# NVlabs/few-shot-vid2vid

Hardware: AMD Instinct MI355X
Metric: frames/sec G+D fwd+bwd step, 512x512 fewshot_pose (higher is better)
Workload: dtype f32; 1 GPU; fewshot_pose 512x512, per-GPU batch 2, adaptive_spade+warp_ref+spade_combine, D step + G step (train.py:58-62), Adam included, no VGG / no FlowNet2 / face-D; global_batch=2, parallelism=dp1, launch=hipgraph

## Files before the change

few-shot-vid2vid_amd/csrc/conv_igemm.hip:

```cpp
#include <stdlib.h>
#include "conv_igemm.h"


__device__ __forceinline__ void fsv_xcd_tile(int nx, int ny, int& bx, int& by) {
  const int b = blockIdx.x + blockIdx.y * nx;
  if ((nx & 7) != 0 || ny == 1) { bx = blockIdx.x; by = blockIdx.y; return; }
  const int xcd = b & 7, j = b >> 3;
  by = j % ny;
  bx = xcd + 8 * (j / ny);
}

template <int BM, int BN, int WM, int WN, int PF, bool AF, int DBG = 0, int MODE = 0, bool UP = false>
__device__ __forceinline__ void fsv_conv_igemm_body(const ConvP& p, const int bx, const int by, const int bz) {
  constexpr bool LD = MODE == 2, WT = MODE >= 1;
  constexpr int BK = FSV_BK;
  constexpr int NT = 64 * WM * WN;
  constexpr int RPA = NT / 8;
  constexpr int TM = BM / (WM * 32), TN = BN / (WN * 32);
  constexpr int NPA = BM / RPA;
  constexpr int QB = BN / 4;
  constexpr int RPB = NT / QB;
  constexpr int NPB = BK / RPB;
  constexpr int A_ST = BM * BK, B_ST = BK * BN;
  static_assert(TM >= 1 && TN >= 1 && NPA >= 1 && NPA * RPA == BM && NPB >= 1 && NPB * RPB == BK, "tile / thread-count mismatch");
// ... 974 lines not shown
      areg[i][0] = fsv_buf_load1(abuf, ok ? (unsigned)(((((long long)n * p.H + iy) * p.W + ix) * p.Cin + ci) * 4) : FSV_BUF_OOB);
    }
#pragma unroll
    for (int i = 0; i < NPB; ++i) {
      int m = pc * BK + bpr0 + i * RPB;
      bool rok = m < p.Mz;
      if (cout4) {
        breg[i] = fsv_buf_load4(bbuf, (rok && bcol < p.Cout) ? (unsigned)((m * p.Cout + bcol) * 4) : FSV_BUF_OOB);
      } else {
        const unsigned e = (unsigned)((m * p.Cout + bcol) * 4);
        breg[i] = make_float4(fsv_buf_load1(bbuf, (rok && bcol + 0 < p.Cout) ? e : FSV_BUF_OOB),
                              fsv_buf_load1(bbuf, (rok && bcol + 1 < p.Cout) ? e + 4 : FSV_BUF_OOB),
                              fsv_buf_load1(bbuf, (rok && bcol + 2 < p.Cout) ? e + 8 : FSV_BUF_OOB),
                              fsv_buf_load1(bbuf, (rok && bcol + 3 < p.Cout) ? e + 12 : FSV_BUF_OOB));
      }
    }
  };
  auto store_chunk = [&]() {
#pragma unroll
    for (int i = 0; i < NPA; ++i) {
      int pr = apr0 + i * RPA;
#pragma unroll
      for (int j = 0; j < V; ++j) As[pr * BMK + aq * V + j] = areg[i][j];
    }
#pragma unroll
    for (int i = 0; i < NPB; ++i) {
      int pr = bpr0 + i * RPB;
      *reinterpret_cast<float4*>(&Bs[pr * BN + bq * 4]) = breg[i];
    }
  };

  f32x16 acc[TM][TN];
#pragma unroll
  for (int i = 0; i < TM; ++i)
#pragma unroll
    for (int j = 0; j < TN; ++j)
#pragma unroll
      for (int r = 0; r < 16; ++r) acc[i][j][r] = 0.f;

  const int lrow = lane & 31, lk = lane >> 5;
  const float* a_frag = &As[lk * BMK + wm * (TM * 32) + lrow];
  const float* b_frag = &Bs[lk * BN + wn * (TN * 32) + lrow];
  if (c_begin < c_end) {
    load_chunk(c_begin);
    store_chunk();
    __syncthreads();
#pragma unroll 1
    for (int pc = c_begin; pc < c_end; ++pc) {
      const int pnext = (pc + 1 < c_end) ? pc + 1 : pc;
      load_chunk(pnext);
      float a[2][TM], b[2][TN];
#pragma unroll
      for (int i = 0; i < TM; ++i) a[0][i] = a_frag[i * 32];
#pragma unroll
      for (int j = 0; j < TN; ++j) b[0][j] = b_frag[j * 32];
#pragma unroll
      for (int kk = 0; kk < BK / 2; ++kk) {
        const int cur = kk & 1, nxt = cur ^ 1;
        if (kk + 1 < BK / 2) {
#pragma unroll
          for (int i = 0; i < TM; ++i) a[nxt][i] = a_frag[(kk + 1) * 2 * BMK + i * 32];
#pragma unroll
          for (int j = 0; j < TN; ++j) b[nxt][j] = b_frag[(kk + 1) * 2 * BN + j * 32];
        }
#pragma unroll
        for (int i = 0; i < TM; ++i)
#pragma unroll
          for (int j = 0; j < TN; ++j)
            acc[i][j] = __builtin_amdgcn_mfma_f32_32x32x2f32(a[cur][i], b[cur][j], acc[i][j], 0, 0, 0);
      }
      __syncthreads();
      store_chunk();
      __syncthreads();
    }
  }
#pragma unroll
  for (int j = 0; j < TN; ++j) {
    const int co = bn0 + wn * (TN * 32) + j * 32 + lrow;
    if (co >= p.Cout) continue;
#pragma unroll
    for (int i = 0; i < TM; ++i)
#pragma unroll
      for (int r = 0; r < 16; ++r) {
        const int row = (r & 3) + 8 * (r >> 2) + 4 * lk;
        const int k = bi0 + wm * (TM * 32) + i * 32 + row;
        if (k >= p.K) continue;
        float* dst = dwt + (long long)k * p.ldw + co;
        if (p.nsplit > 1) atomicAdd(dst, acc[i][j][r]); else *dst = acc[i][j][r];
      }
  }
}

#define FSV_THIN_MAXK 1152
template <int CO>
__global__ __launch_bounds__(256) void fsv_conv_thin_fwd_kernel(ConvP p, int iters) {
  __shared__ float wl[FSV_THIN_MAXK * CO];
  const int tid = threadIdx.x, lane = tid & 63, wave = tid >> 6;
  for (int i = tid; i < p.K * CO; i += 256) {
    const int k = i / CO, c = i - k * CO;
    wl[i] = (c < p.Cout) ? p.wt[(long long)k * p.ldw + c] : 0.f;
  }
  __syncthreads();
  const int QC = p.Cin >> 2;
  const int PPW = 64 / QC;
  const int cq = lane % QC, pl = lane / QC;
  const int ohw = p.OH * p.OW;
  const fsv_buf abuf = fsv_make_buf(p.in, (long long)p.N * p.H * p.W * p.Cin * 4);
  const float ws = p.wscale ? p.wscale[0] : 1.f;
  const int m_base = blockIdx.x * (4 * PPW * iters);
#pragma unroll 1
  for (int it = 0; it < iters; ++it) {
    const int m = m_base + (it * 4 + wave) * PPW + pl;
    const bool live = m < p.Mz;
    const int mm = live ? m : 0;
    const int n = mm / ohw, rem = mm - n * ohw;
    const int oy = rem / p.OW, ox = rem - oy * p.OW;
    float acc[CO];
#pragma unroll
    for (int c = 0; c < CO; ++c) acc[c] = 0.f;
#pragma unroll 3
    for (int t = 0; t < p.ntaps; ++t) {
      int ty, tx;
      fsv_tap(p, t, ty, tx);
      const int iy = oy * p.sy + ty, ix = ox * p.sx + tx;
      const bool ok = live & ((unsigned)iy < (unsigned)p.H) & ((unsigned)ix < (unsigned)p.W);
      const float4 v = fsv_buf_load4(abuf, ok ? (unsigned)((((n * p.H + iy) * p.W + ix) * p.Cin + cq * 4) * 4) : FSV_BUF_OOB);
      const float* w0 = wl + (t * p.Cin + cq * 4) * CO;
#pragma unroll
      for (int c = 0; c < CO; ++c) {
        acc[c] = fmaf(v.x, w0[c], acc[c]);
        acc[c] = fmaf(v.y, w0[CO + c], acc[c]);
        acc[c] = fmaf(v.z, w0[2 * CO + c], acc[c]);
        acc[c] = fmaf(v.w, w0[3 * CO + c], acc[c]);
      }
    }
    for (int o = 1; o < QC; o <<= 1) {
#pragma unroll
      for (int c = 0; c < CO; ++c) acc[c] += __shfl_xor(acc[c], o);
    }
    if (live && cq == 0) {
#pragma unroll
      for (int c = 0; c < CO; ++c) {
        if (c >= p.Cout) break;
        float v = acc[c] * ws;
        v = (v + (p.bias ? p.bias[c] : 0.f)) * p.scale;
        v = fsv_act(v, p.act);
        if (p.res) v += p.res[(long long)m * p.Cout + c];
        p.out[(long long)m * p.Cout + c] = v;
      }
    }
  }
}

template <int CO>
__global__ __launch_bounds__(256) void fsv_conv_thin_wgrad_kernel(WgradP p, int chunk) {
  __shared__ float red[256 * 4 * CO];
  const int QK = p.ntaps * (p.Cin >> 2);
  const int NG = 256 / QK;
  const int tid = threadIdx.x;
  const int q = tid % QK, g = tid / QK;
  const bool lane_on = g < NG;
  const int t = q / (p.Cin >> 2), ci = (q - t * (p.Cin >> 2)) * 4;
  int ty, tx;
  {
    unsigned long long code = (t < 8) ? p.taps_lo : p.taps_hi;
    int sh = (t & 7) * 8;
    ty = (int)((code >> sh) & 15ull) - 8;
    tx = (int)((code >> (sh + 4)) & 15ull) - 8;
  }
  const fsv_buf abuf = fsv_make_buf(p.in, (long long)p.N * p.H * p.W * p.Cin * 4);
  const fsv_buf dbuf = fsv_make_buf(p.dout, (long long)p.Mz * p.Cout * 4);
  const int ohw = p.OH * p.OW;
  const int m0 = blockIdx.x * chunk;
  const int m1 = (m0 + chunk < p.Mz) ? m0 + chunk : p.Mz;
  float acc[4][CO];
#pragma unroll
  for (int e = 0; e < 4; ++e)
#pragma unroll
    for (int c = 0; c < CO; ++c) acc[e][c] = 0.f;
  if (lane_on) {
#pragma unroll 4
    for (int m = m0 + g; m < m1; m += NG) {
      const int n = m / ohw, rem = m - n * ohw;
      const int oy = rem / p.OW, ox = rem - oy * p.OW;
      const int iy = oy * p.sy + ty, ix = ox * p.sx + tx;
      const bool ok = ((unsigned)iy < (unsigned)p.H) & ((unsigned)ix < (unsigned)p.W);
      const float4 v = fsv_buf_load4(abuf, ok ? (unsigned)((((n * p.H + iy) * p.W + ix) * p.Cin + ci) * 4) : FSV_BUF_OOB);
      float d[CO];
#pragma unroll
      for (int c = 0; c < CO; ++c) d[c] = fsv_buf_load1(dbuf, (c < p.Cout) ? (unsigned)((m * p.Cout + c) * 4) : FSV_BUF_OOB);
#pragma unroll
      for (int c = 0; c < CO; ++c) {
        acc[0][c] = fmaf(v.x, d[c], acc[0][c]);
        acc[1][c] = fmaf(v.y, d[c], acc[1][c]);
        acc[2][c] = fmaf(v.z, d[c], acc[2][c]);
        acc[3][c] = fmaf(v.w, d[c], acc[3][c]);
      }
    }
  }
#pragma unroll
  for (int e = 0; e < 4; ++e)
#pragma unroll
    for (int c = 0; c < CO; ++c) red[(e * CO + c) * 256 + tid] = acc[e][c];
  __syncthreads();
  if (g == 0) {
#pragma unroll
    for (int e = 0; e < 4; ++e)
#pragma unroll
      for (int c = 0; c < CO; ++c) {
        float s = 0.f;
        for (int gg = 0; gg < NG; ++gg) s += red[(e * CO + c) * 256 + gg * QK + q];
        if (c < p.Cout) atomicAdd(p.dwt + (long long)(t * p.Cin + ci + e) * p.ldw + c, s);
      }
  }
}

static inline bool fsv_conv_thin(int Mz, int K) {
  const int sw = (int)fsv_env("FSV_CONV_THIN", 1);
  if (sw == 0) return false;
  if (sw == 2) return true;
  return K <= 1152 && (long long)Mz >= 64ll * K;
}

__global__ __launch_bounds__(256) void fsv_prep_weight_kernel(const float* w, float* wt, const float* scale_ptr,
                                                              const float* col_scale,
                                                              int mode_in, int Cout, int Cin, int KH, int KW,
                                                              int ntaps, unsigned long long taps_lo,
                                                              unsigned long long taps_hi, int Kpad, int ldw,
                                                              long long w_bstride, long long wt_bstride) {
  const int z = blockIdx.z;
  const float s = scale_ptr ? *scale_ptr : 1.f;
  const long long total = (long long)Kpad * ldw;
  const bool accum = mode_in == 3;
  const int mode = accum ? 2 : mode_in;
  const int rowlen = (mode == 1) ? Cout : Cin;
  const int ncols = (mode == 1) ? Cin : Cout;
  const int K = ntaps * rowlen;
  long long i = (long long)blockIdx.x * 256 + threadIdx.x;
  const long long stride = (long long)gridDim.x * 256;
  for (; i < total; i += stride) {
    int r = (int)(i / ldw), c = (int)(i - (long long)r * ldw);
    bool ok = r < K && c < ncols;
    int j = ok ? r / rowlen : 0;
    int a = r - j * rowlen;
    unsigned long long code = (j < 8) ? taps_lo : taps_hi;
    int sh = (j & 7) * 8;
    int kh = (int)((code >> sh) & 15ull), kw = (int)((code >> (sh + 4)) & 15ull);
    int co = (mode == 1) ? a : c, ci = (mode == 1) ? c : a;
    long long widx = (((long long)co * Cin + ci) * KH + kh) * KW + kw + (long long)z * w_bstride;
    if (mode == 2) {
      if (ok) {
        float g = s * wt[(long long)z * wt_bstride + i];
        ((float*)w)[widx] = accum ? ((float*)w)[widx] + g : g;
      }
    } else {
      float v = 0.f;
      if (ok) v = col_scale ? w[widx] * col_scale[co] : s * w[widx];
      wt[(long long)z * wt_bstride + i] = v;
    }
  }
}

struct PrepGroup {
  const long long* src; const long long* dst; const int* dims; const unsigned long long* taps;
};
template <int KKT>
__device__ __forceinline__ void fsv_prep_stage(const PrepGroup& g, const int layer, const int cot, const int cit, float* t) {
  const int* d = g.dims + layer * 9;
  const int Cout = d[0], CinR = d[2], KW = d[4];
  const int KK = KKT ? KKT : d[3] * KW;
  const int CI_T = KK <= 8 ? 32 : 16;
  const int run = CI_T * KK, lds = run + 1;
  const float* w = reinterpret_cast<const float*>(g.src[layer]);
  const int co0 = cot * 32, ci0 = cit * CI_T;
  const int tid = threadIdx.x;
  const int total = 32 * run;
  constexpr int U = 8;
  for (int e0 = tid; e0 < total; e0 += 256 * U) {
    float val[U];
    int dst[U];
#pragma unroll
    for (int u = 0; u < U; ++u) {
      const int e = e0 + 256 * u;
      const int col = e / run, idx = e - col * run;
      const int co = co0 + col, ci = ci0 + idx / KK;
      const bool ok = (e < total) & (co < Cout) & (ci < CinR);
      val[u] = ok ? w[((long long)co * CinR + ci0) * KK + idx] : 0.f;
      dst[u] = (e < total) ? col * lds + idx : -1;
    }
#pragma unroll
    for (int u = 0; u < U; ++u)
      if (dst[u] >= 0) t[dst[u]] = val[u];
  }
}

__device__ __forceinline__ float fsv_prep_pick(const float* src, const int code, const int KW, const bool masked) {
  if (!masked) return src[(code & 15) * KW + (code >> 4)];
  const int mh = code & 15, mw = code >> 4;
  float s = 0.f;
  bool first = true;
  for (int kh = 0; kh < 4; ++kh) {
    if (!((mh >> kh) & 1)) continue;
    for (int kw = 0; kw < 4; ++kw) {
      if (!((mw >> kw) & 1)) continue;
      const float v = src[kh * KW + kw];
      s = first ? v : s + v;
      first = false;
    }
  }
  return s;
}

template <int KKT>
__device__ __forceinline__ void fsv_prep_emit(const PrepGroup& g, const int layer, const int cot, const int cit, const float* t) {
  const int* d = g.dims + layer * 9;
  const int Cout = d[0], CinP = d[1], KW = d[4], ntaps = d[5], ldw = d[7];
  const int mode = d[8] & 1;
  const bool masked = (d[8] & 4) != 0;
  const int KK = KKT ? KKT : d[3] * KW;
  const int CI_T = KK <= 8 ? 32 : 16;
  const int run = CI_T * KK, lds = run + 1;
  float* wt = reinterpret_cast<float*>(g.dst[layer]);
  const unsigned long long lo = g.taps[layer * 2], hi = g.taps[layer * 2 + 1];
  const int co0 = cot * 32, ci0 = cit * CI_T;
  const int tid = threadIdx.x;
  if (mode == 0) {
    const int q = tid & 7, r0 = tid >> 3;
    const int nrows = ntaps * CI_T;
    for (int r = r0; r < nrows; r += 32) {
      const int j = r / CI_T, cil = r - j * CI_T;
      const int ci = ci0 + cil;
      if (ci >= CinP) continue;
      const unsigned long long code8 = (j < 8) ? lo : hi;
      const int code = (int)((code8 >> ((j & 7) * 8)) & 255ull);
      const float* src = t + (4 * q) * lds + cil * KK;
      *reinterpret_cast<float4*>(&wt[((long long)j * CinP + ci) * ldw + co0 + 4 * q]) =
          make_float4(fsv_prep_pick(src, code, KW, masked), fsv_prep_pick(src + lds, code, KW, masked),
                      fsv_prep_pick(src + 2 * lds, code, KW, masked), fsv_prep_pick(src + 3 * lds, code, KW, masked));
    }
  } else {
    const int QN = CI_T / 4;
    const int q = tid % QN, r0 = tid / QN, rstep = 256 / QN;
    const int nrows = ntaps * 32;
    for (int r = r0; r < nrows; r += rstep) {
      const int j = r >> 5, col = r & 31;
      const int co = co0 + col, ci = ci0 + 4 * q;
      if (co >= Cout || ci >= CinP) continue;
      const unsigned long long code8 = (j < 8) ? lo : hi;
      const int code = (int)((code8 >> ((j & 7) * 8)) & 255ull);
      const float* src = t + col * lds + (4 * q) * KK;
      float* dstp = &wt[((long long)j * Cout + co) * ldw + ci];
      if (ci + 3 < CinP) {
        *reinterpret_cast<float4*>(dstp) =
            make_float4(fsv_prep_pick(src, code, KW, masked), fsv_prep_pick(src + KK, code, KW, masked),
                        fsv_prep_pick(src + 2 * KK, code, KW, masked), fsv_prep_pick(src + 3 * KK, code, KW, masked));
      } else {
        for (int k = 0; ci + k < CinP; ++k) dstp[k] = fsv_prep_pick(src + k * KK, code, KW, masked);
      }
    }
  }
}

template <int KKT>
__device__ __forceinline__ void fsv_prep_layer(const PrepGroup& g, const int first, const int njobs, const int cot, const int cit,
                                               float* t) {
  fsv_prep_stage<KKT>(g, first, cot, cit, t);
  __syncthreads();
  for (int j = 0; j < njobs; ++j) fsv_prep_emit<KKT>(g, first + j, cot, cit, t);
}

__global__ __launch_bounds__(256) void fsv_prep_group_kernel(PrepGroup g, const int* tmap) {
  __shared__ float t[32 * 257];
  const int first = tmap[blockIdx.x * 4], njobs = tmap[blockIdx.x * 4 + 1];
  const int cot = tmap[blockIdx.x * 4 + 2], cit = tmap[blockIdx.x * 4 + 3];
// ... 112 lines not shown
      FSV_CONV_TILES(FSV_V4_CASE)
      FSV_CONV_TILES_DIAG(FSV_V4_CASE)
#undef FSV_V4_CASE
      default: return FSV_ERR_BAD_ARG;
    }
  } else {
    switch (t->shape) {
#define FSV_V1_CASE(SHAPE, BM, BN, WM, WN) \
  case SHAPE: FSV_LAUNCH((fsv_conv_igemm_v1_kernel<BM, BN, WM, WN>), g, dim3(64 * WM * WN), stream, p); break;
      FSV_CONV_V1_SHAPES(FSV_V1_CASE)
#undef FSV_V1_CASE
      default: return FSV_ERR_BAD_ARG;
    }
  }
  return fsv_check_launch();
}

#include <stdlib.h>
#include <string.h>
static inline long long fsv_tune(int which) {
  static long long vals[4] = {-1, -1, -1, -1};
  if (vals[0] < 0) {
    vals[1] = (long long)fsv_env("FSV_SPLIT_TARGET", 512);
    vals[2] = (long long)fsv_env("FSV_WG_TARGET", 1024);
    vals[3] = (long long)fsv_env("FSV_WG_MINCH", 8);
    vals[0] = (long long)fsv_env("FSV_SPLIT_BELOW", 256);
  }
  return vals[which];
}

static inline double fsv_conv_cost(int Mz, int Cout, int nchunks, int nsamp, int tile, int nsplit) {
  const FsvTile* row = fsv_tile_row(tile);
  if (!row) return 1e30;
  const int bm = row->bm, bn = row->bn;
  const bool w8 = row->wm * row->wn >= 8;
  const double wgs = (double)fsv_cdiv(Mz, bm) * fsv_cdiv(Cout, bn) * nsamp * nsplit;
  const double L = (double)((long long)((wgs + 255.0) / 256.0));
  const double cps = (double)fsv_cdiv(nchunks, nsplit);
  const double cyc = (double)bm * bn / 4.0;
  const double eff = w8 ? (L <= 1.0 ? 0.91 : 0.97) : (L <= 1.0 ? 0.78 : (L <= 2.0 ? 0.88 : 0.95));
  const double ovh = (5000.0 + bm * bn / 8.0) * (L <= 1.0 ? 1.0 : 0.45);
  double t = L * (cps * cyc / eff + ovh) / 1.95e9 + 4e-6;
  static double split_fix = -1.0, split_bw = 0.0;
  if (split_fix < 0.0) {
    split_bw = fsv_env("FSV_SPLIT_BW_TBS", 4.5) * 1e12;
    split_fix = fsv_env("FSV_SPLIT_FIX_US", 3.0) * 1e-6;
  }
  if (nsplit > 1) t += split_fix + 0.5e-6 * nsplit + (double)Mz * Cout * nsamp * 4.0 * (2.0 + 0.25 * nsplit) / split_bw;
  return t;
}

template <class F>
static inline void fsv_plan_candidates(int cout, int only, F visit) {
  static const int tiles[5] = {0, 9, 1, 4, 2};
  for (int ti = 0; ti < 5; ++ti) {
    const int t = tiles[ti];
    if (only >= 0 ? t != only : (((t == 0 || t == 9) && cout <= 64) || (t == 1 && cout <= 32) || (t == 2 && cout > 32))) continue;
    visit(t, 1.0 + 0.01 * ti);
  }
}

static inline bool fsv_deterministic() {
  return fsv_env("FSV_DETERMINISTIC", 0) == 1;
}

extern "C" int fsv_conv_thin_rule(int Mz, int K) { return fsv_conv_thin(Mz, K) ? 1 : 0; }

extern "C" int fsv_conv_plan(int Mz, int Cout, int nchunks, int nsamp, int force_tile, int force_split,
                             int* tile_out, int* nsplit_out) {
  if (force_split <= 0 && fsv_deterministic()) force_split = 1;
  int tile = force_tile, nsplit = force_split > 0 ? force_split : 1;
  if (tile < 0 || force_split <= 0) {
    static const int splits[6] = {1, 2, 3, 4, 6, 8};
    double best = 1e30;
    int bt = -1, bs = 1;
    fsv_plan_candidates(Cout, force_tile, [&](int t, double weight) {
      for (int si = 0; si < 6; ++si) {
        const int sp = splits[si];
        if (force_split > 0 && sp != 1) break;
        const int use = force_split > 0 ? force_split : sp;
        if (use > 1 && nchunks / use < 8) break;
        const double c = fsv_conv_cost(Mz, Cout, nchunks, nsamp, t, use) * weight;
        if (c < best) { best = c; bt = t; bs = use; }
      }
    });
    if (bt < 0) { bt = force_tile >= 0 ? force_tile : (Cout <= 32 ? 2 : 4); bs = force_split > 0 ? force_split : 1; }
    tile = bt; nsplit = bs;
  }
  if (!fsv_tile_row(tile)) return -1;
  if (nsplit > nchunks) nsplit = nchunks;
  if (nsplit < 1) nsplit = 1;
  *tile_out = tile; *nsplit_out = nsplit;
  return 0;
}

static inline void fsv_fill_convp(ConvP& p, const float* in, const float* wt, const float* bias, const float* res, float* out,
                                  const float* wscale, int N, int H, int W, int Cin, int OH, int OW, int Cout, int ntaps,
                                  const int* ty, const int* tx, int sy, int sx, int outH, int outW, int osy, int osx, int ooy,
                                  int oox, int ldw, long long w_bstride, long long b_bstride, int per_sample, int act,
                                  float scale) {
  p.in = in; p.wt = wt; p.bias = bias; p.res = res; p.out = out; p.wscale = wscale;
  p.N = N; p.H = H; p.W = W; p.Cin = Cin; p.OH = OH; p.OW = OW; p.Cout = Cout;
  p.K = ntaps * Cin; p.nchunks = fsv_cdiv(p.K, FSV_BK); p.ldw = ldw;
  p.sy = sy; p.sx = sx; p.ntaps = ntaps;
  fsv_pack_taps(ty, tx, ntaps, p.taps_lo, p.taps_hi, 8);
  p.outH = outH; p.outW = outW; p.osy = osy; p.osx = osx; p.ooy = ooy; p.oox = oox;
  p.dense_out = (osy == 1 && osx == 1 && ooy == 0 && oox == 0 && outH == OH && outW == OW) ? 1 : 0;
  p.w_bstride = w_bstride; p.b_bstride = b_bstride; p.per_sample = per_sample ? 1 : 0;
  p.act = act; p.scale = scale;
  p.Mz = per_sample ? OH * OW : N * OH * OW;
  p.nsplit = 1;
  p.stats = nullptr; p.stats_slots = 1; p.stats_ohw = 1;
  p.part = nullptr; p.part_stride = 0;
  p.up = 0;
  {
    const long long obytes = (long long)N * outH * outW * Cout * 4;
    p.res_bytes = (res && obytes <= FSV_BUF_MAX_BYTES) ? obytes : 0;
  }
}

static inline bool vec4_ok(int cin) { return (cin & 3) == 0; }

static inline int fsv_conv_check_args(const float* in, const float* wt, const float* out, int N, int H, int W, int Cin, int Cout,
                                      int ntaps, const int* ty, const int* tx, int ldw) {
  if (!in || !wt || !out || ntaps < 1 || ntaps > 16 || N < 1 || Cin < 1 || Cout < 1) return FSV_ERR_BAD_ARG;
  for (int t = 0; t < ntaps; ++t)
    if (ty[t] < -8 || ty[t] > 7 || tx[t] < -8 || tx[t] > 7) return FSV_ERR_UNSUPPORTED;
  if ((ldw & 3) != 0 || ldw < Cout) return FSV_ERR_BAD_ARG;
  if ((long long)N * H * W * Cin * 4 > FSV_BUF_MAX_BYTES || (long long)(ntaps * Cin + 32) * ldw * 4 > FSV_BUF_MAX_BYTES) return FSV_ERR_UNSUPPORTED;
  return FSV_OK;
}

static int fsv_conv_gather_impl(const float* in, const float* wt, const float* bias, const float* res, float* out,
                        int N, int H, int W, int Cin, int OH, int OW, int Cout,
                        int ntaps, const int* ty, const int* tx, int sy, int sx,
                        int outH, int outW, int osy, int osx, int ooy, int oox,
                        int ldw, long long w_bstride, long long b_bstride, int per_sample,
                        int act, float scale, int force_tile, int force_split, int accumulate, const float* wscale,
                        double* stats, int stats_groups, int stats_slots, int stats_prezeroed, int* produced,
                        float* split_ws, long long split_cap, int in_up, hipStream_t stream) {
  if (const int bad = fsv_conv_check_args(in, wt, out, N, H, W, Cin, Cout, ntaps, ty, tx, ldw)) return bad;
  if (in_up && ((H & 1) || (W & 1) || (Cin % 4 != 0) || per_sample || accumulate || Cout <= 4)) return FSV_ERR_UNSUPPORTED;
  ConvP p;
  fsv_fill_convp(p, in, wt, bias, res, out, wscale, N, H, W, Cin, OH, OW, Cout, ntaps, ty, tx, sy, sx, outH, outW, osy, osx, ooy,
                 oox, ldw, w_bstride, b_bstride, per_sample, act, scale);
  p.up = in_up ? 1 : 0;
  const int nsamp = per_sample ? N : 1;
  int tile = 0, nsplit = 1;
  if (Cout <= 4 && (Cin % 4 == 0) && Cin <= 256 && ((Cin >> 2) & ((Cin >> 2) - 1)) == 0 && p.K <= FSV_THIN_MAXK && !per_sample &&
      p.dense_out && !accumulate && force_tile < 0 && force_split <= 0 && !stats &&
      act != FSV_ACT_DLRELU && fsv_conv_thin(p.Mz, p.K)) {
    p.nsplit = 1;
    if (produced) *produced = 0;
    const int ppb = 4 * (64 / (Cin >> 2));
    int iters = 16;
    while (iters > 1 && fsv_cdiv(p.Mz, ppb * iters) < 1024) iters >>= 1;
    const dim3 g(fsv_cdiv(p.Mz, ppb * iters));
    switch (Cout) {
      case 1: FSV_LAUNCH((fsv_conv_thin_fwd_kernel<1>), g, dim3(256), stream, p, iters); break;
      case 2: FSV_LAUNCH((fsv_conv_thin_fwd_kernel<2>), g, dim3(256), stream, p, iters); break;
      case 3: FSV_LAUNCH((fsv_conv_thin_fwd_kernel<3>), g, dim3(256), stream, p, iters); break;
      default: FSV_LAUNCH((fsv_conv_thin_fwd_kernel<4>), g, dim3(256), stream, p, iters); break;
    }
    return fsv_check_launch();
  }
  if (act == FSV_ACT_DLRELU) {
    if (!res || accumulate) return FSV_ERR_BAD_ARG;
    force_split = 1;
  }
  if (fsv_conv_plan(p.Mz, Cout, p.nchunks, nsamp, force_tile, force_split, &tile, &nsplit)) return FSV_ERR_BAD_ARG;
  p.nsplit = nsplit;
  const long long total = (long long)N * outH * outW * Cout;
  if (accumulate) {
    if (bias || res || act != FSV_ACT_NONE || scale != 1.f) return FSV_ERR_BAD_ARG;
  } else if (nsplit > 1) {
    if (!p.dense_out) return FSV_ERR_UNSUPPORTED;
    if (split_ws && (Cin % 4 == 0) && split_cap >= (long long)nsplit * total) {
      p.part = split_ws; p.part_stride = total;
    } else {
      (void)hipMemsetAsync(out, 0, (size_t)total * sizeof(float), stream);
    }
  }
  const bool vec4 = (Cin % 4 == 0);
  if (produced) *produced = 0;
  if (stats && vec4 && nsplit == 1 && !accumulate && !per_sample && p.dense_out && stats_groups >= 1 && stats_slots >= 1 &&
      p.Mz % stats_groups == 0 && (stats_groups == 1 || p.Mz / stats_groups >= 128)) {
    p.stats = stats; p.stats_slots = stats_slots; p.stats_ohw = p.Mz / stats_groups;
    if (!stats_prezeroed)
      (void)hipMemsetAsync(stats, 0, (size_t)stats_groups * stats_slots * Cout * 2 * sizeof(double), stream);
    if (produced) *produced = 1;
  }
  double* fin_stats = nullptr;
  {
    if (stats && fsv_env("FSV_SPLIT_FIN_STATS", 1) != 0 && fsv_env("FSV_SPLIT_FIN4", 1) != 0 && nsplit > 1 && p.part && !accumulate && !per_sample && p.dense_out &&
        stats_groups >= 1 && stats_slots >= 1 && (Cout % 32) == 0 && p.Mz % stats_groups == 0 && ((p.Mz / stats_groups) % 32) == 0 &&
        act != FSV_ACT_DLRELU && !fsv_deterministic() &&
        (((unsigned long long)p.part | (unsigned long long)out | (unsigned long long)res) & 15ull) == 0) {
      fin_stats = stats;
      if (!stats_prezeroed)
        (void)hipMemsetAsync(stats, 0, (size_t)stats_groups * stats_slots * Cout * 2 * sizeof(double), stream);
      if (produced) *produced = 1;
    }
  }
  if (force_tile < 0 && vec4) tile = fsv_conv_variant(tile);
  int rc = fsv_launch_conv(p, vec4, nsamp * nsplit, stream, tile);
  if (rc) return rc;
  if (!accumulate && nsplit > 1 && (p.part || bias || res || act != FSV_ACT_NONE || scale != 1.f)) {
    int grid = (int)((total + 256 * 8 - 1) / (256 * 8));
    if (grid > 4096) grid = 4096;
    if (grid < 1) grid = 1;
    const bool fin4 = fsv_env("FSV_SPLIT_FIN4", 1) != 0 && p.part && (Cout % 4 == 0) && (total % 4 == 0) &&
                      (((unsigned long long)p.part | (unsigned long long)out | (unsigned long long)res) & 15ull) == 0;
    if (fin_stats) {
      const long long npix = (long long)N * outH * outW;
      FSV_LAUNCH(fsv_split_finish4_stats_kernel, dim3((unsigned)((npix + 31) / 32), (unsigned)(Cout / 32)), dim3(256), stream,
                 (const float4*)p.part, p.part_stride / 4, nsplit, (float4*)out, bias, (const float4*)res, npix, Cout, act, scale,
                 fin_stats, stats_slots, (long long)(p.Mz / stats_groups));
    } else if (fin4) {
      int g4 = (int)((total / 4 + 255) / 256);
      if (g4 > 8192) g4 = 8192;
      FSV_LAUNCH(fsv_split_finish4_kernel, dim3(g4), dim3(256), stream, (const float4*)p.part, p.part_stride / 4, nsplit, (float4*)out,
                 bias, (const float4*)res, total / 4, Cout, (long long)outH * outW, per_sample ? b_bstride : 0ll, act, scale);
    } else if (p.part)
      FSV_LAUNCH(fsv_split_finish_kernel, dim3(grid), dim3(256), stream, (const float*)p.part, p.part_stride, nsplit, out, bias, res,
                 total, Cout, (long long)outH * outW, per_sample ? b_bstride : 0ll, act, scale);
    else
      FSV_LAUNCH(fsv_bias_act_kernel, dim3(grid), dim3(256), stream, out, bias, res, total, Cout,
                 (long long)outH * outW, per_sample ? b_bstride : 0ll, act, scale);
    rc = fsv_check_launch();
  }
  return rc;
}

extern "C" {

int fsv_conv_gather_fwd(const float* in, const float* wt, const float* bias, const float* res, float* out,
                        int N, int H, int W, int Cin, int OH, int OW, int Cout,
                        int ntaps, const int* ty, const int* tx, int sy, int sx,
                        int outH, int outW, int osy, int osx, int ooy, int oox,
                        int ldw, long long w_bstride, long long b_bstride, int per_sample,
                        int act, float scale, int force_tile, int force_split, int accumulate, const float* wscale,
                        float* split_ws, long long split_ws_floats, int in_up, hipStream_t stream) {
  return fsv_conv_gather_impl(in, wt, bias, res, out, N, H, W, Cin, OH, OW, Cout, ntaps, ty, tx, sy, sx, outH, outW, osy, osx,
                              ooy, oox, ldw, w_bstride, b_bstride, per_sample, act, scale, force_tile, force_split, accumulate,
                              wscale, nullptr, 0, 0, 0, nullptr, split_ws, split_ws ? split_ws_floats : 0, in_up, stream);
}

int fsv_conv_gather_fwd_stats(const float* in, const float* wt, const float* bias, const float* res, float* out,
                              int N, int H, int W, int Cin, int OH, int OW, int Cout,
                              int ntaps, const int* ty, const int* tx, int sy, int sx,
                              int ldw, int act, float scale, const float* wscale,
                              double* stats, int stats_groups, int stats_slots, int stats_prezeroed, int* produced,
                              float* split_ws, long long split_ws_floats, int in_up, hipStream_t stream) {
  if (!stats || !produced) return FSV_ERR_BAD_ARG;
  return fsv_conv_gather_impl(in, wt, bias, res, out, N, H, W, Cin, OH, OW, Cout, ntaps, ty, tx, sy, sx, OH, OW, 1, 1, 0, 0, ldw,
                              0, 0, 0, act, scale, -1, 0, 0, wscale, stats, stats_groups, stats_slots, stats_prezeroed, produced,
                              split_ws, split_ws ? split_ws_floats : 0, in_up, stream);
}

int fsv_bias_act(float* x, const float* bias, long long total, int C, int act, hipStream_t stream) {
  if (!x || total < 1 || C < 1) return FSV_ERR_BAD_ARG;
  int grid = (int)((total + 256 * 8 - 1) / (256 * 8));
  if (grid > 4096) grid = 4096;
  if (grid < 1) grid = 1;
  FSV_LAUNCH(fsv_bias_act_kernel, dim3(grid), dim3(256), stream, x, bias, (const float*)nullptr, total, C, 1ll, 0ll, act,
             1.f);
  return fsv_check_launch();
}

}

static inline void fsv_fill_wgradp(WgradP& p, const float* in, const float* dout, float* dwt, int N, int H, int W, int Cin, int OH,
                                   int OW, int Cout, int ntaps, const int* ty, const int* tx, int sy, int sx, int ldw,
                                   long long w_bstride, int per_sample, int in_up) {
  p.in = in; p.dout = dout; p.dwt = dwt;
  p.N = N; p.H = H; p.W = W; p.Cin = Cin; p.OH = OH; p.OW = OW; p.Cout = Cout;
  p.K = ntaps * Cin; p.ldw = ldw; p.sy = sy; p.sx = sx; p.ntaps = ntaps;
  fsv_pack_taps(ty, tx, ntaps, p.taps_lo, p.taps_hi, 8);
  p.w_bstride = w_bstride; p.per_sample = per_sample ? 1 : 0;
  p.Mz = per_sample ? OH * OW : N * OH * OW;
  p.pchunks = fsv_cdiv(p.Mz, FSV_BK);
  p.up = in_up ? 1 : 0;
}

extern "C" {

int fsv_conv_wgrad(const float* in, const float* dout, float* dwt,
                   int N, int H, int W, int Cin, int OH, int OW, int Cout,
                   int ntaps, const int* ty, const int* tx, int sy, int sx,
                   int ldw, int Kpad, long long w_bstride, int per_sample, int force_split, int prezeroed,
                   int force_tile, int in_up, hipStream_t stream) {
  if (!in || !dout || !dwt || ntaps < 1 || ntaps > 16) return FSV_ERR_BAD_ARG;
  if (in_up && ((H & 1) || (W & 1) || (Cin % 4 != 0) || (Cout & 3) != 0 || Cout <= 4 || per_sample || FSV_BK / OW + 1 > OH))
    return FSV_ERR_UNSUPPORTED;
  for (int t = 0; t < ntaps; ++t)
    if (ty[t] < -8 || ty[t] > 7 || tx[t] < -8 || tx[t] > 7) return FSV_ERR_UNSUPPORTED;
  if ((long long)N * H * W * Cin * 4 > FSV_BUF_MAX_BYTES || (long long)N * OH * OW * Cout * 4 > FSV_BUF_MAX_BYTES) return FSV_ERR_UNSUPPORTED;
  WgradP p;
  fsv_fill_wgradp(p, in, dout, dwt, N, H, W, Cin, OH, OW, Cout, ntaps, ty, tx, sy, sx, ldw, w_bstride, per_sample, in_up);
  const int nsamp = per_sample ? N : 1;
  if (Cout <= 4 && vec4_ok(Cin) && !per_sample && force_tile == 0 && force_split <= 0 && ntaps * (Cin >> 2) <= 256 &&
      fsv_conv_thin(p.Mz, p.K) && (!fsv_deterministic() || (int)fsv_env("FSV_CONV_THIN", 1) == 2)) {
    p.nsplit = 1;
    if (!prezeroed) (void)hipMemsetAsync(dwt, 0, (size_t)Kpad * ldw * sizeof(float), stream);
    int chunk = fsv_cdiv(p.Mz, 512);
    if (chunk < 64) chunk = 64;
    const dim3 g(fsv_cdiv(p.Mz, chunk));
    switch (Cout) {
      case 1: FSV_LAUNCH((fsv_conv_thin_wgrad_kernel<1>), g, dim3(256), stream, p, chunk); break;
      case 2: FSV_LAUNCH((fsv_conv_thin_wgrad_kernel<2>), g, dim3(256), stream, p, chunk); break;
      case 3: FSV_LAUNCH((fsv_conv_thin_wgrad_kernel<3>), g, dim3(256), stream, p, chunk); break;
      default: FSV_LAUNCH((fsv_conv_thin_wgrad_kernel<4>), g, dim3(256), stream, p, chunk); break;
    }
    return fsv_check_launch();
  }
  int bn = (Cout <= 32) ? 32 : (Cout <= 64 ? 64 : 128);
  int bmk = 128;
  if (vec4_ok(Cin) && bn >= 64) bmk = (p.K <= 32) ? 32 : (p.K <= 64 ? 64 : 128);
  if (force_tile == 1 && vec4_ok(Cin) && Cout > 32) { bmk = 64; bn = 64; }
  else if (force_tile == 2 && vec4_ok(Cin) && Cout > 32) { bmk = 128; bn = 64; }
  else if (force_tile == 3 && vec4_ok(Cin) && Cout > 64) { bmk = 64; bn = 128; }
  else if (force_tile == 4 && vec4_ok(Cin) && Cout > 64) { bmk = 128; bn = 128; }
  long long target = fsv_tune(2);
  static int wplan_v = -1;
  if (wplan_v < 0) wplan_v = (int)fsv_env("FSV_WGRAD_PLAN", 1);
  if (force_tile == 0 && wplan_v == 1 && vec4_ok(Cin) && Cout >= 64 && p.K > 64) {
    bmk = 64; bn = 64; target = 2048;
  }
  long long blocks = (long long)fsv_cdiv(p.K, bmk) * fsv_cdiv(Cout, bn) * nsamp;
  int nsplit = 1;
  if (force_split > 0) nsplit = force_split;
  else if (fsv_deterministic()) nsplit = 1;
  else {
    nsplit = (int)((target + blocks - 1) / blocks);
    int maxs = p.pchunks / (int)fsv_tune(3);
    if (nsplit > maxs) nsplit = maxs;
    if (nsplit < 1) nsplit = 1;
  }
  if (nsplit > p.pchunks) nsplit = p.pchunks;
  p.nsplit = nsplit;
  if (nsplit > 1 && !prezeroed)
    (void)hipMemsetAsync(dwt, 0, (size_t)((per_sample ? (long long)N * w_bstride : (long long)Kpad * ldw)) * sizeof(float), stream);
  dim3 block(256);
  const bool vec4 = (Cin % 4 == 0) && (FSV_BK / OW + 1 <= OH) && ((Cout & 3) == 0 || bn == 32);
  dim3 g(fsv_cdiv(p.K, bmk), fsv_cdiv(Cout, bn), nsamp * nsplit);
  if (vec4) {
    if (bn == 128 && bmk == 32) FSV_LAUNCH((fsv_conv_wgrad_kernel<32, 128, 1, 4, true>), g, block, stream, p);
    else if (bn == 128 && bmk == 64) FSV_LAUNCH((fsv_conv_wgrad_kernel<64, 128, 2, 2, true>), g, block, stream, p);
    else if (bn == 64 && bmk == 32) FSV_LAUNCH((fsv_conv_wgrad_kernel<32, 64, 1, 2, true>), g, dim3(128), stream, p);
    else if (bn == 64 && bmk == 64) FSV_LAUNCH((fsv_conv_wgrad_kernel<64, 64, 2, 2, true>), g, block, stream, p);
    else if (bn == 128) FSV_LAUNCH((fsv_conv_wgrad_kernel<128, 128, 2, 2, true>), g, block, stream, p);
    else if (bn == 64) FSV_LAUNCH((fsv_conv_wgrad_kernel<128, 64, 2, 2, true>), g, block, stream, p);
    else if ((Cout & 3) == 0) FSV_LAUNCH((fsv_conv_wgrad_kernel<128, 32, 4, 1, true>), g, block, stream, p);
    else FSV_LAUNCH((fsv_conv_wgrad_kernel<128, 32, 4, 1, false>), g, block, stream, p);
  } else {
    if (bn == 128) FSV_LAUNCH((fsv_conv_wgrad_v1_kernel<128, 128, 2, 2>), g, block, stream, p);
    else if (bn == 64) FSV_LAUNCH((fsv_conv_wgrad_v1_kernel<128, 64, 2, 2>), g, block, stream, p);
    else FSV_LAUNCH((fsv_conv_wgrad_v1_kernel<128, 32, 4, 1>), g, block, stream, p);
  }
  return fsv_check_launch();
}

int fsv_prep_weight(const float* w, float* wt, const float* scale_ptr, int mode, int nbatch,
                    int Cout, int Cin, int KH, int KW, int ntaps, const int* kh, const int* kw,
                    int Kpad, int ldw, long long w_bstride, long long wt_bstride, const float* col_scale, hipStream_t stream) {
  if (!w || !wt || ntaps < 1 || ntaps > 16 || mode < 0 || mode > 3) return FSV_ERR_BAD_ARG;
  if (col_scale && (scale_ptr || mode != 0)) return FSV_ERR_BAD_ARG;
  unsigned long long lo, hi;
  fsv_pack_taps(kh, kw, ntaps, lo, hi, 0);
  long long total = (long long)Kpad * ldw;
  int grid = (int)((total + 255) / 256);
  if (grid > 2048) grid = 2048;
  FSV_LAUNCH(fsv_prep_weight_kernel, dim3(grid, 1, nbatch), dim3(256), stream, w, wt, scale_ptr, col_scale, mode, Cout,
             Cin, KH, KW, ntaps, lo, hi, Kpad, ldw, w_bstride, wt_bstride);
  return fsv_check_launch();
}


static inline double fsv_group_cost(const ConvP* ps, const int* nsamp, int n, int tile) {
  const FsvTile* row = fsv_tile_row(tile);
  if (!row) return 1e30;
  const int bm = row->bm, bn = row->bn;
  const bool w8 = row->wm * row->wn >= 8;
  const double cyc = (double)bm * bn / 4.0;
  const double ovh = 5000.0 + bm * bn / 8.0;
  double load = 0.0, crit = 0.0;
  for (int i = 0; i < n; ++i) {
    const double wgs = (double)fsv_cdiv(ps[i].Mz, bm) * fsv_cdiv(ps[i].Cout, bn) * nsamp[i];
    const double one = ps[i].nchunks * cyc;
    load += wgs * (one / 0.95 + 0.45 * ovh);
    const double lone = one / (w8 ? 0.91 : 0.78) + ovh;
    if (lone > crit) crit = lone;
  }
  load /= 256.0;
  return (load > crit ? load : crit) / 1.95e9 + 4e-6;
}

static inline int fsv_group_tile(const ConvP* ps, const int* nsamp, int n) {
  int max_cout = 0;
  for (int i = 0; i < n; ++i)
    if (ps[i].Cout > max_cout) max_cout = ps[i].Cout;
  double best = 1e30;
  int tile = 4;
  fsv_plan_candidates(max_cout, -1, [&](int t, double weight) {
    const double c = fsv_group_cost(ps, nsamp, n, t) * weight;
    if (c < best) { best = c; tile = t; }
  });
  return tile;
}

static inline void fsv_group_order(const long long* weight, int n, int* order) {
  for (int i = 0; i < n; ++i) order[i] = i;
  for (int i = 1; i < n; ++i) {
    const int v = order[i];
    int j = i - 1;
    while (j >= 0 && weight[order[j]] < weight[v]) { order[j + 1] = order[j]; --j; }
    order[j + 1] = v;
  }
}

#define FSV_GROUP_LIMIT 64

int fsv_conv_gather_group(const fsv_conv_desc* d, int n, int force_tile, hipStream_t stream) {
  if (!d || n < 1 || n > FSV_GROUP_LIMIT) return FSV_ERR_BAD_ARG;
  ConvP ps[FSV_GROUP_LIMIT];
  int nsamp[FSV_GROUP_LIMIT];
  long long weight[FSV_GROUP_LIMIT];
  bool vec4 = true;
  for (int i = 0; i < n; ++i) {
    const fsv_conv_desc& q = d[i];
    if (const int bad = fsv_conv_check_args(q.in, q.wt, q.out, q.N, q.H, q.W, q.Cin, q.Cout, q.ntaps, q.ty, q.tx, q.ldw)) return bad;
    if (q.accumulate && (q.bias || q.res || q.act != FSV_ACT_NONE || q.scale != 1.f)) return FSV_ERR_BAD_ARG;
    if (q.act == FSV_ACT_DLRELU && !q.res) return FSV_ERR_BAD_ARG;
    fsv_fill_convp(ps[i], q.in, q.wt, q.bias, q.res, q.out, q.wscale, q.N, q.H, q.W, q.Cin, q.OH, q.OW, q.Cout, q.ntaps, q.ty,
                   q.tx, q.sy, q.sx, q.outH, q.outW, q.osy, q.osx, q.ooy, q.oox, q.ldw, q.w_bstride, q.b_bstride, q.per_sample,
                   q.act, q.scale);
    nsamp[i] = q.per_sample ? q.N : 1;
    vec4 = vec4 && vec4_ok(q.Cin);
  }
  const FsvTile* row = fsv_tile_row(force_tile < 0 ? fsv_group_tile(ps, nsamp, n) : force_tile);
  if (!row) return FSV_ERR_BAD_ARG;
  const int tile = row->shape, bm = row->bm, bn = row->bn;
  long long wgs1 = 0;
  for (int i = 0; i < n; ++i) wgs1 += (long long)fsv_cdiv(ps[i].Mz, bm) * fsv_cdiv(ps[i].Cout, bn) * nsamp[i];
  int want = 1;
  if (wgs1 <= 384 && !fsv_deterministic()) { want = (int)((768 + wgs1 - 1) / (wgs1 > 0 ? wgs1 : 1)); if (want > 8) want = 8; if (want < 1) want = 1; }
  for (int i = 0; i < n; ++i) {
    int sp = 1;
    if (d[i].accumulate && want > 1) {
      sp = want;
      if (sp > ps[i].nchunks / 8) sp = ps[i].nchunks / 8;
      if (sp < 1) sp = 1;
    }
    ps[i].nsplit = sp;
    weight[i] = (long long)fsv_cdiv(ps[i].nchunks, sp);
  }
  int order[FSV_GROUP_LIMIT];
// ... 102 lines not shown
```

Baseline: 47.55 frames/s.

## Add LDS-tiled halo-patch kernels for thin-output conv forward and wgrad

Result: no change. 47.79 frames/s (median of 6 runs) (+0.5%).

```diff
diff --git a/few-shot-vid2vid_amd/csrc/conv_igemm.hip b/few-shot-vid2vid_amd/csrc/conv_igemm.hip
--- a/few-shot-vid2vid_amd/csrc/conv_igemm.hip
+++ b/few-shot-vid2vid_amd/csrc/conv_igemm.hip
@@ -1150,6 +1150,146 @@
   }
 }
 
+#define FSV_THIN_TH 8
+#define FSV_THIN_PATCH_Q 2880
+struct ThinTile { int TW, lw, tiles_x, tiles_y, ntiles; };
+
+static inline bool fsv_thin_tiled_geom(int Cin, int Cout, int ntaps, const int* ty, const int* tx, int sy, int sx) {
+  if (sy != 1 || sx != 1 || Cin > 64 || Cin % 4 != 0 || ((Cin >> 2) & ((Cin >> 2) - 1)) != 0 || (ntaps != 9 && ntaps != 1) ||
+      ntaps * 4 * Cout > 144)
+    return false;
+  for (int t = 0; t < ntaps; ++t)
+    if (ty[t] < -1 || ty[t] > 1 || tx[t] < -1 || tx[t] > 1) return false;
+  return true;
+}
+
+static inline ThinTile fsv_thin_tile(int N, int OH, int OW, int Cin) {
+  ThinTile tt;
+  tt.TW = Cin > 32 ? 16 : 32; tt.lw = Cin > 32 ? 4 : 5;
+  tt.tiles_x = fsv_cdiv(OW, tt.TW); tt.tiles_y = fsv_cdiv(OH, FSV_THIN_TH);
+  tt.ntiles = N * tt.tiles_x * tt.tiles_y;
+  return tt;
+}
+
+__device__ __forceinline__ void fsv_thin_stage(float* patch, const fsv_rawbuf araw, int n, int y0, int x0, int H, int W, int Cin,
+                                               int PH, int PW, int tid) {
+  const int QC = Cin >> 2;
+  const int rowq = PW * QC, total = PH * rowq;
+  const int lane = tid & 63;
+  for (int i0 = tid - lane; i0 < total; i0 += 256) {
+    const int i = i0 + lane;
+    const int r = i / rowq, c4 = i - r * rowq;
+    const int c = c4 / QC, q = c4 - c * QC;
+    const int gy = y0 + r, gx = x0 + c;
+    const bool ok = (i < total) & ((unsigned)gy < (unsigned)H) & ((unsigned)gx < (unsigned)W);
+    fsv_buf_load4_lds(araw, ok ? (unsigned)((((n * H + gy) * W + gx) * Cin + q * 4) * 4) : FSV_BUF_OOB, patch + i0 * 4);
+  }
+}
+
+template <int O>
+__device__ __forceinline__ float fsv_fold_lane(float v) {
+#ifdef FSV_EMU
+  return __shfl_xor(v, O);
+#else
+  constexpr int ctrl = O == 1 ? 0xB1 : (O == 2 ? 0x4E : (O == 4 ? 0x141 : 0x140));
+  return __builtin_bit_cast(float, __builtin_amdgcn_update_dpp(0, __builtin_bit_cast(int, v), ctrl, 0xF, 0xF, false));
+#endif
+}
+
+template <int CO, int NT>
+__global__ __launch_bounds__(256) void fsv_conv_thin_tiled_fwd_kernel(ConvP p, ThinTile tt) {
+  __shared__ __attribute__((aligned(16))) float4 patch[FSV_THIN_PATCH_Q];
+  __shared__ float sums[FSV_THIN_TH * 32 * CO];
+  const int tid = threadIdx.x, lane = tid & 63, wave = tid >> 6;
+  const int QC = p.Cin >> 2;
+  const int PPW = 64 / QC;
+  const int cq = lane % QC, pl = lane / QC;
+  int miny = 1, maxy = -1, minx = 1, maxx = -1;
+  int tys[NT], txs[NT];
+#pragma unroll
+  for (int t = 0; t < NT; ++t) {
+    fsv_tap(p, t, tys[t], txs[t]);
+    miny = tys[t] < miny ? tys[t] : miny; maxy = tys[t] > maxy ? tys[t] : maxy;
+    minx = txs[t] < minx ? txs[t] : minx; maxx = txs[t] > maxx ? txs[t] : maxx;
+  }
+  const int PH = FSV_THIN_TH + maxy - miny, PW = tt.TW + maxx - minx;
+  float w[NT][4][CO];
+  int toff[NT];
+#pragma unroll
+  for (int t = 0; t < NT; ++t) {
+    toff[t] = ((tys[t] - miny) * PW + (txs[t] - minx)) * QC;
+#pragma unroll
+    for (int e = 0; e < 4; ++e)
+#pragma unroll
+      for (int c = 0; c < CO; ++c)
+        w[t][e][c] = (c < p.Cout) ? p.wt[(long long)(t * p.Cin + cq * 4 + e) * p.ldw + c] : 0.f;
+  }
+  const fsv_rawbuf araw = fsv_make_rawbuf(p.in, (long long)p.N * p.H * p.W * p.Cin * 4);
+  const float ws = p.wscale ? p.wscale[0] : 1.f;
+  float bs[CO];
+#pragma unroll
+  for (int c = 0; c < CO; ++c) bs[c] = (p.bias && c < p.Cout) ? p.bias[c] : 0.f;
+  const int npix = FSV_THIN_TH * tt.TW;
+  const int iters = npix / (4 * PPW);
+  const int tpi = tt.tiles_x * tt.tiles_y;
+#pragma unroll 1
+  for (int tile = blockIdx.x; tile < tt.ntiles; tile += gridDim.x) {
+    const int n = tile / tpi, tr = tile - n * tpi;
+    const int tyi = tr / tt.tiles_x, txi = tr - tyi * tt.tiles_x;
+    const int y0 = tyi * FSV_THIN_TH, x0 = txi * tt.TW;
+    fsv_thin_stage(reinterpret_cast<float*>(patch), araw, n, y0 + miny, x0 + minx, p.H, p.W, p.Cin, PH, PW, tid);
+    FSV_WAIT_VMCNT(0);
+    __syncthreads();
+#pragma unroll 1
+    for (int it = 0; it < iters; ++it) {
+      const int tp = (it * 4 + wave) * PPW + pl;
+      const int py = tp >> tt.lw, px = tp & (tt.TW - 1);
+      const float4* src = patch + (py * PW + px) * QC + cq;
+      float acc[CO];
+#pragma unroll
+      for (int c = 0; c < CO; ++c) acc[c] = 0.f;
+#pragma unroll
+      for (int t = 0; t < NT; ++t) {
+        const float4 v = src[toff[t]];
+#pragma unroll
+        for (int c = 0; c < CO; ++c) {
+          acc[c] = fmaf(v.x, w[t][0][c], acc[c]);
+          acc[c] = fmaf(v.y, w[t][1][c], acc[c]);
+          acc[c] = fmaf(v.z, w[t][2][c], acc[c]);
+          acc[c] = fmaf(v.w, w[t][3][c], acc[c]);
+        }
+      }
+#pragma unroll
+      for (int c = 0; c < CO; ++c) {
+        if (QC > 1) acc[c] += fsv_fold_lane<1>(acc[c]);
+        if (QC > 2) acc[c] += fsv_fold_lane<2>(acc[c]);
+        if (QC > 4) acc[c] += fsv_fold_lane<4>(acc[c]);
+        if (QC > 8) acc[c] += fsv_fold_lane<8>(acc[c]);
+      }
+      if (cq == 0) {
+#pragma unroll
+        for (int c = 0; c < CO; ++c) sums[tp * CO + c] = acc[c];
+      }
+    }
+    __syncthreads();
+    if (tid < npix) {
+      const int oy = y0 + (tid >> tt.lw), ox = x0 + (tid & (tt.TW - 1));
+      if ((oy < p.OH) & (ox < p.OW)) {
+        const long long m = ((long long)n * p.OH + oy) * p.OW + ox;
+#pragma unroll
+        for (int c = 0; c < CO; ++c) {
+          if (c >= p.Cout) break;
+          float v = sums[tid * CO + c] * ws;
+          v = (v + bs[c]) * p.scale;
+          v = fsv_act(v, p.act);
+          if (p.res) v += p.res[m * p.Cout + c];
+          p.out[m * p.Cout + c] = v;
+        }
+      }
+    }
+  }
+}
+
 template <int CO>
 __global__ __launch_bounds__(256) void fsv_conv_thin_wgrad_kernel(WgradP p, int chunk) {
   __shared__ float red[256 * 4 * CO];
@@ -1213,11 +1353,103 @@
   }
 }
 
+template <int CO>
+__global__ __launch_bounds__(256) void fsv_conv_thin_tiled_wgrad_kernel(WgradP p, ThinTile tt) {
+  __shared__ __attribute__((aligned(16))) float4 patch[FSV_THIN_PATCH_Q];
+  __shared__ __attribute__((aligned(16))) float4 dq[FSV_THIN_TH * 32];
+  static_assert(256 * 4 * CO * 4 <= FSV_THIN_PATCH_Q * 16, "the fold re-uses the patch");
+  float* const red = reinterpret_cast<float*>(patch);
+  const int QC = p.Cin >> 2;
+  const int QK = p.ntaps * QC;
+  const int NG = 256 / QK;
+  const int tid = threadIdx.x;
+  const int q = tid % QK, g = tid / QK;
+  const bool lane_on = g < NG;
+  const int t = q / QC, cq = q - t * QC, ci = cq * 4;
+  int miny = 1, maxy = -1, minx = 1, maxx = -1, ty = 0, tx = 0;
+  for (int tt_ = 0; tt_ < p.ntaps; ++tt_) {
+    const unsigned long long code = (tt_ < 8) ? p.taps_lo : p.taps_hi;
+    const int sh = (tt_ & 7) * 8;
+    const int y = (int)((code >> sh) & 15ull) - 8, x = (int)((code >> (sh + 4)) & 15ull) - 8;
+    miny = y < miny ? y : miny; maxy = y > maxy ? y : maxy;
+    minx = x < minx ? x : minx; maxx = x > maxx ? x : maxx;
+    if (tt_ == t) { ty = y; tx = x; }
+  }
+  const int PH = FSV_THIN_TH + maxy - miny, PW = tt.TW + maxx - minx;
+  const int loff = ((ty - miny) * PW + (tx - minx)) * QC + cq;
+  const fsv_rawbuf araw = fsv_make_rawbuf(p.in, (long long)p.N * p.H * p.W * p.Cin * 4);
+  const fsv_buf dbuf = fsv_make_buf(p.dout, (long long)p.Mz * p.Cout * 4);
+  const int npix = FSV_THIN_TH * tt.TW;
+  const int tpi = tt.tiles_x * tt.tiles_y;
+  float acc[4][CO];
+#pragma unroll
+  for (int e = 0; e < 4; ++e)
+#pragma unroll
+    for (int c = 0; c < CO; ++c) acc[e][c] = 0.f;
+#pragma unroll 1
+  for (int tile = blockIdx.x; tile < tt.ntiles; tile += gridDim.x) {
+    const int n = tile / tpi, tr = tile - n * tpi;
+    const int tyi = tr / tt.tiles_x, txi = tr - tyi * tt.tiles_x;
+    const int y0 = tyi * FSV_THIN_TH, x0 = txi * tt.TW;
+    fsv_thin_stage(reinterpret_cast<float*>(patch), araw, n, y0 + miny, x0 + minx, p.H, p.W, p.Cin, PH, PW, tid);
+    if (tid < npix) {
+      const int oy = y0 + (tid >> tt.lw), ox = x0 + (tid & (tt.TW - 1));
+      const bool live = (oy < p.OH) & (ox < p.OW);
+      const int m = (n * p.OH + oy) * p.OW + ox;
+      float d[4];
+#pragma unroll
+      for (int c = 0; c < 4; ++c) d[c] = fsv_buf_load1(dbuf, (live && c < p.Cout) ? (unsigned)((m * p.Cout + c) * 4) : FSV_BUF_OOB);
+      dq[tid] = make_float4(d[0], d[1], d[2], d[3]);
+    }
+    FSV_WAIT_VMCNT(0);
+    __syncthreads();
+    if (lane_on) {
+      const int rows = (p.OH - y0 < FSV_THIN_TH) ? p.OH - y0 : FSV_THIN_TH;
+#pragma unroll 4
+      for (int pix = g; pix < rows * tt.TW; pix += NG) {
+        const int py = pix >> tt.lw, px = pix & (tt.TW - 1);
+        const float4 v = patch[(py * PW + px) * QC + loff];
+        const float4 dv = dq[pix];
+        const float d[4] = {dv.x, dv.y, dv.z, dv.w};
+#pragma unroll
+        for (int c = 0; c < CO; ++c) {
+          acc[0][c] = fmaf(v.x, d[c], acc[0][c]);
+          acc[1][c] = fmaf(v.y, d[c], acc[1][c]);
+          acc[2][c] = fmaf(v.z, d[c], acc[2][c]);
+          acc[3][c] = fmaf(v.w, d[c], acc[3][c]);
+        }
+      }
+    }
+    __syncthreads();
+  }
+#pragma unroll
+  for (int e = 0; e < 4; ++e)
+#pragma unroll
+    for (int c = 0; c < CO; ++c) red[(e * CO + c) * 256 + tid] = acc[e][c];
+  __syncthreads();
+  if (g == 0) {
+#pragma unroll
+    for (int e = 0; e < 4; ++e)
+#pragma unroll
+      for (int c = 0; c < CO; ++c) {
+        float s = 0.f;
+        for (int gg = 0; gg < NG; ++gg) s += red[(e * CO + c) * 256 + gg * QK + q];
+        if (c < p.Cout) atomicAdd(p.dwt + (long long)(t * p.Cin + ci + e) * p.ldw + c, s);
+      }
+  }
+}
+
 static inline bool fsv_conv_thin(int Mz, int K) {
   const int sw = (int)fsv_env("FSV_CONV_THIN", 1);
   if (sw == 0) return false;
-  if (sw == 2) return true;
+  if (sw == 2 || sw == 3) return true;
   return K <= 1152 && (long long)Mz >= 64ll * K;
+}
+static inline bool fsv_conv_thin_tiled() { return (int)fsv_env("FSV_CONV_THIN", 1) != 3; }
+
+static inline int fsv_thin_tiled_grid(int ntiles, int cap) {
+  const int rounds = fsv_cdiv(ntiles, cap);
+  return fsv_cdiv(ntiles, rounds);
 }
 
 __global__ __launch_bounds__(256) void fsv_prep_weight_kernel(const float* w, float* wt, const float* scale_ptr,
@@ -1636,6 +1868,21 @@
       act != FSV_ACT_DLRELU && fsv_conv_thin(p.Mz, p.K)) {
     p.nsplit = 1;
     if (produced) *produced = 0;
+    if (fsv_conv_thin_tiled() && fsv_thin_tiled_geom(Cin, Cout, ntaps, ty, tx, sy, sx) && ntaps * 4 * Cout <= 108) {
+      const ThinTile tt = fsv_thin_tile(N, OH, OW, Cin);
+      const dim3 g(fsv_thin_tiled_grid(tt.ntiles, 768));
+#define FSV_THIN_TILED_FWD(CO)                                                                                        \
+  if (ntaps == 1) FSV_LAUNCH((fsv_conv_thin_tiled_fwd_kernel<CO, 1>), g, dim3(256), stream, p, tt);                   \
+  else FSV_LAUNCH((fsv_conv_thin_tiled_fwd_kernel<CO, 9>), g, dim3(256), stream, p, tt)
+      switch (Cout) {
+        case 1: FSV_THIN_TILED_FWD(1); break;
+        case 2: FSV_THIN_TILED_FWD(2); break;
+        case 3: FSV_THIN_TILED_FWD(3); break;
+        default: FSV_LAUNCH((fsv_conv_thin_tiled_fwd_kernel<4, 1>), g, dim3(256), stream, p, tt); break;
+      }
+#undef FSV_THIN_TILED_FWD
+      return fsv_check_launch();
+    }
     const int ppb = 4 * (64 / (Cin >> 2));
     int iters = 16;
     while (iters > 1 && fsv_cdiv(p.Mz, ppb * iters) < 1024) iters >>= 1;
@@ -1784,9 +2031,20 @@
   fsv_fill_wgradp(p, in, dout, dwt, N, H, W, Cin, OH, OW, Cout, ntaps, ty, tx, sy, sx, ldw, w_bstride, per_sample, in_up);
   const int nsamp = per_sample ? N : 1;
   if (Cout <= 4 && vec4_ok(Cin) && !per_sample && force_tile == 0 && force_split <= 0 && ntaps * (Cin >> 2) <= 256 &&
-      fsv_conv_thin(p.Mz, p.K) && (!fsv_deterministic() || (int)fsv_env("FSV_CONV_THIN", 1) == 2)) {
+      fsv_conv_thin(p.Mz, p.K) && (!fsv_deterministic() || (int)fsv_env("FSV_CONV_THIN", 1) >= 2)) {
     p.nsplit = 1;
     if (!prezeroed) (void)hipMemsetAsync(dwt, 0, (size_t)Kpad * ldw * sizeof(float), stream);
+    if (fsv_conv_thin_tiled() && fsv_thin_tiled_geom(Cin, Cout, ntaps, ty, tx, sy, sx)) {
+      const ThinTile tt = fsv_thin_tile(N, OH, OW, Cin);
+      const dim3 g(fsv_thin_tiled_grid(tt.ntiles, 512));
+      switch (Cout) {
+        case 1: FSV_LAUNCH((fsv_conv_thin_tiled_wgrad_kernel<1>), g, dim3(256), stream, p, tt); break;
+        case 2: FSV_LAUNCH((fsv_conv_thin_tiled_wgrad_kernel<2>), g, dim3(256), stream, p, tt); break;
+        case 3: FSV_LAUNCH((fsv_conv_thin_tiled_wgrad_kernel<3>), g, dim3(256), stream, p, tt); break;
+        default: FSV_LAUNCH((fsv_conv_thin_tiled_wgrad_kernel<4>), g, dim3(256), stream, p, tt); break;
+      }
+      return fsv_check_launch();
+    }
     int chunk = fsv_cdiv(p.Mz, 512);
     if (chunk < 64) chunk = 64;
     const dim3 g(fsv_cdiv(p.Mz, chunk));
```
